# Fantom-foundation/go-txflow

Measured on AMD Instinct MI355X. Metric: verified+tallied TxVotes/sec, higher is better.
Workload: dtype u32

## Files before the change

### go-txflow_amd/csrc/fe10.h

```cpp
#pragma once
#include "fe.h"

namespace txv {

struct fe10 { uint32_t v[10]; };

#define TXV_W10(i) (((i) & 1) ? 25 : 26)
#define TXV_M10(i) (((i) & 1) ? 0x1ffffffu : 0x3ffffffu)

TXV_HD uint32_t fe10_2p(int i) { return i == 0 ? 0x7ffffdau : ((i & 1) ? 0x3fffffeu : 0x7fffffeu); }

TXV_HD fe10 fe10_zero() { fe10 r; for (int i = 0; i < 10; ++i) r.v[i] = 0; return r; }
TXV_HD fe10 fe10_one() { fe10 r = fe10_zero(); r.v[0] = 1; return r; }

TXV_HD fe10 fe10_add(const fe10& a, const fe10& b) {
  fe10 r;
#pragma unroll
  for (int i = 0; i < 10; ++i) r.v[i] = a.v[i] + b.v[i];
  return r;
}
TXV_HD fe10 fe10_sub(const fe10& a, const fe10& b) {
  fe10 r;
#pragma unroll
  for (int i = 0; i < 10; ++i) r.v[i] = (a.v[i] + fe10_2p(i)) - b.v[i];
// ... 191 lines not shown
  }
  const uint32_t t = r.v[0] + 19u * c;
  r.v[0] = t & 0x3ffffffu;
  r.v[1] += t >> 26;
  return r;
}

TXV_HD fe10 fe10_from_fe(const fe& a) {
  fe10 r;
  const uint32_t top = a.v[7] >> 31;
  int bit = 0;
#pragma unroll
  for (int i = 0; i < 10; ++i) {
    const int w = bit >> 5, s = bit & 31;
    uint32_t x = a.v[w] >> s;
    if (s + TXV_W10(i) > 32 && w < 7) x |= a.v[w + 1] << (32 - s);
    r.v[i] = x & TXV_M10(i);
    bit += TXV_W10(i);
  }
  r.v[0] += 19u * top;
  return r;
}

TXV_HD fe fe_from_fe10(const fe10& a) {
  const fe10 s = fe10_strict(a);
  fe r;
#pragma unroll
  for (int w = 0; w < 8; ++w) r.v[w] = 0;
  int bit = 0;
#pragma unroll
  for (int i = 0; i < 10; ++i) {
    const int w = bit >> 5, sh = bit & 31;
    r.v[w] |= s.v[i] << sh;
    if (sh + TXV_W10(i) > 32 && w < 7) r.v[w + 1] |= s.v[i] >> (32 - sh);
    bit += TXV_W10(i);
  }
  return r;
}

}
```

### go-txflow_amd/csrc/fe_inv_var.h

```cpp
#pragma once
#include "fe.h"

namespace txv {

struct s30 { int32_t v[9]; };

constexpr int32_t kM30 = 0x3FFFFFFF;
TXV_HD int32_t p30(int i) { return i == 0 ? 0x3FFFFFED : (i == 8 ? 0x7FFF : 0x3FFFFFFF); }
constexpr uint32_t inv30_p() {
  uint32_t p0 = 0x3FFFFFEDu, x = p0;
  for (int i = 0; i < 5; ++i) x *= 2u - p0 * x;
  return x & 0x3FFFFFFFu;
}
constexpr uint32_t kPInv30 = inv30_p();
static_assert((0x3FFFFFEDu * kPInv30 & 0x3FFFFFFFu) == 1u, "p^-1 mod 2^30");

TXV_HD uint32_t inv256_odd(uint32_t f) {
  uint32_t x = f;
  x *= 2u - f * x;
  x *= 2u - f * x;
  return x;
}

TXV_HD int32_t divsteps30_var(int32_t eta, uint32_t f, uint32_t g, int32_t t[4]) {
  uint32_t u = 1, v = 0, q = 0, r = 1;
  int i = 30;
  for (;;) {
    const int zeros = __builtin_ctz(g | (0xFFFFFFFFu << i));
    g >>= zeros; u <<= zeros; v <<= zeros; eta -= zeros; i -= zeros;
    if (i == 0) break;
    if (eta < 0) {
      uint32_t tmp;
      eta = -eta;
      tmp = f; f = g; g = 0u - tmp;
      tmp = u; u = q; q = 0u - tmp;
      tmp = v; v = r; r = 0u - tmp;
    }
    const int limit = (eta + 1) > i ? i : (eta + 1);
    const uint32_t m = (0xFFFFFFFFu >> (32 - limit)) & 255u;
    const uint32_t w = (g * inv256_odd(f)) & m;
    g -= f * w; q -= u * w; r -= v * w;
  }
// ... 100 lines not shown
```

### go-txflow_amd/csrc/ge.h

```cpp
#pragma once
#include "fe.h"
#include "fe10.h"

namespace txv {

struct ge_ext { fe X, Y, Z, T; };
struct ge_niels { fe ypx, ymx, xy2d; };

TXV_HD ge_ext ge_identity() {
  ge_ext r; r.X = fe_zero(); r.Y = fe_one(); r.Z = fe_one(); r.T = fe_zero(); return r;
}

struct ge10_ext { fe10 X, Y, Z, T; };

TXV_HD ge10_ext ge10_madd(const ge10_ext& p, const fe10& qp, const fe10& qm, const fe10& qd, bool neg) {
  const fe10 C = fe10_cneg(fe10_mul(p.T, qd), neg);
  TXV_SCHED_FENCE();
  const fe10 A = fe10_mul(fe10_sub(p.Y, p.X), qm);
  TXV_SCHED_FENCE();
  const fe10 B = fe10_mul(fe10_add(p.Y, p.X), qp);
  TXV_SCHED_FENCE();
  const fe10 E = fe10_sub(B, A), H = fe10_add(B, A);
  const fe10 G = fe10_add(p.Z, C), F = fe10_sub(p.Z, C);
  ge10_ext r;
// ... 122 lines not shown
  ge_ext r;
  r.X = fe_mul(E, F); r.Y = fe_mul(G, H); r.Z = fe_mul(F, G); r.T = fe_mul(E, H);
  return r;
}

TXV_HD ge_ext ge_dbl(const ge_ext& p) {
  fe A = fe_sq(p.X), B = fe_sq(p.Y), C = fe_dbl(fe_sq(p.Z));
  fe AB = fe_add(A, B);
  fe E = fe_sub(fe_sq(fe_add(p.X, p.Y)), AB);
  fe G = fe_sub(B, A);
  fe H = fe_neg(AB);
  fe F = fe_sub(G, C);
  ge_ext r;
  r.X = fe_mul(E, F); r.Y = fe_mul(G, H); r.Z = fe_mul(F, G); r.T = fe_mul(E, H);
  return r;
}

TXV_HD void ge_encode_zinv(uint32_t out[8], const fe& X, const fe& Y, const fe& zi) {
  fe x = fe_canon(fe_mul(X, zi));
  fe y = fe_canon(fe_mul(Y, zi));
#pragma unroll
  for (int i = 0; i < 8; ++i) out[i] = y.v[i];
  out[7] |= (x.v[0] & 1u) << 31;
}
TXV_HD void ge_encode(uint32_t out[8], const ge_ext& p) { ge_encode_zinv(out, p.X, p.Y, fe_invert(p.Z)); }

TXV_HD bool ge_decode(ge_ext& h, const uint32_t w[8]) {
  fe one = fe_one();
  h.Y = fe_from_words_255(w);
  h.Z = one;
  fe u = fe_sq(h.Y);
  fe v = fe_mul(u, fe_const_d());
  u = fe_sub(u, one);
  v = fe_add(v, one);
  fe v3 = fe_mul(fe_sq(v), v);
  fe x = fe_mul(fe_mul(fe_sq(v3), v), u);
  x = fe_pow22523(x);
  x = fe_mul(fe_mul(x, v3), u);
  fe vxx = fe_mul(fe_sq(x), v);
  bool ok = true;
  if (!fe_iszero(fe_sub(vxx, u))) {
    if (!fe_iszero(fe_add(vxx, u))) ok = false;
    x = fe_mul(x, fe_const_sqrtm1());
  }
  if (fe_parity(x) != (w[7] >> 31)) x = fe_neg(x);
  h.X = x;
// ... 15 lines not shown
```

### go-txflow_amd/csrc/kernels_verify.hip

```cpp
#include <algorithm>
#include <cstdlib>

#include "ed25519_dev.h"
#include "fe_inv_var.h"
#include "txv_device.h"

using namespace txv;

#ifndef TXV_K1A_PREFETCH
#define TXV_K1A_PREFETCH 0
#endif

#ifndef TXV_INV_VAR
#define TXV_INV_VAR 1
#endif
__device__ __forceinline__ fe verify_invert(const fe& z) {
#if TXV_INV_VAR
  return fe_invert_var(z);
#else
  return fe_invert(z);
#endif
}

template <int W>
__global__ void __launch_bounds__(64) txv_k_build_tables(const uint32_t* __restrict__ pubs_le, uint32_t n_points,
                                                          uint32_t* __restrict__ tables,
                                                          uint8_t* __restrict__ decode_ok,
                                                          uint32_t* __restrict__ addr_words,
                                                          const uint32_t* __restrict__ out_slot) {
  constexpr int chunks = (Tab<W>::kEntries - 1) / 8;
  constexpr uint64_t per_point = Tab<W>::kBuildLanes;
  const uint64_t gid = (uint64_t)blockIdx.x * 64 + threadIdx.x;
  const uint32_t pt = (uint32_t)(gid / per_point);
  const int t = (int)(gid % per_point);
  if (pt >= n_points) return;
  constexpr int last = Tab<W>::kPositions - 1;
  const bool top = Tab<W>::kLongTop && t >= last * chunks;
  const int pos = top ? last : t / chunks, c = top ? t - last * chunks : t % chunks;
  uint32_t w[8];
#pragma unroll
  for (int i = 0; i < 8; ++i) w[i] = pubs_le[pt * 8 + i];
  if (t == 0 && addr_words) {
    uint32_t h[8];
    sha256_32bytes(h, w);
#pragma unroll
// ... 59 lines not shown
                                                              uint32_t s_out[8]) {
  return vote_challenge(a, i, k_out, s_out);
}

__device__ __forceinline__ bool vote_checks(const VerifyArgs& a, uint32_t i, uint32_t s[16], uint64_t pre[8]) {
  const uint8_t fl = a.flags[i];
  const uint32_t v = a.val[i];
#pragma unroll
  for (int j = 0; j < 16; ++j) s[j] = a.sig[(size_t)j * a.n_pad + i];
  const bool bad = !(fl & TXV_FLAG_PENDING) || !(fl & TXV_FLAG_SIG64) || (fl & TXV_FLAG_BADMSG) ||
                   (s[15] & 0xE0000000u) || !a.decode_ok[v] || !sc_lt_L(s + 8);
  const uint32_t* pw = a.pubs_le + (size_t)v * 8;
#pragma unroll
  for (int j = 0; j < 4; ++j) {
    pre[j] = be64_from_le32(s[2 * j], s[2 * j + 1]);
    pre[4 + j] = be64_from_le32(pw[2 * j], pw[2 * j + 1]);
  }
  return !bad;
}

__global__ void __launch_bounds__(256, 2) txv_k_challenge2(VerifyArgs a) {
  const uint32_t half = (a.n + 1) / 2;
  const uint32_t t = blockIdx.x * 256 + threadIdx.x;
  if (t >= half) return;
  const uint32_t i0 = t, i1 = t + half;
  const bool has1 = i1 < a.n;
  uint32_t s0[16], s1[16];
  uint64_t p0[8], p1[8];
  const bool ok0 = vote_checks(a, i0, s0, p0);
  const bool ok1 = has1 && vote_checks(a, has1 ? i1 : i0, s1, p1);
  if (!ok0 && !ok1) {
    a.ok_out[i0] = 0;
    if (has1) a.ok_out[i1] = 0;
    return;
  }
  const uint32_t j1 = has1 ? i1 : i0;
  MsgView m0{a.msg + i0, a.n_pad, a.msg_words, a.msg_len[i0]};
  MsgView m1{a.msg + j1, a.n_pad, a.msg_words, a.msg_len[j1]};
  uint32_t d0[16], d1[16];
  sha512_prefixed2(d0, p0, m0, d1, p1, m1, 8);
  if (ok0) {
    const sc k = sc_reduce512(d0);
#pragma unroll
    for (int j = 0; j < 8; ++j) a.kbuf[(size_t)j * a.n_pad + i0] = k.v[j];
  }
  a.ok_out[i0] = ok0 ? 2 : 0;
  if (has1) {
    if (ok1) {
      const sc k = sc_reduce512(d1);
#pragma unroll
      for (int j = 0; j < 8; ++j) a.kbuf[(size_t)j * a.n_pad + i1] = k.v[j];
    }
    a.ok_out[i1] = ok1 ? 2 : 0;
  }
}

#ifndef TXV_K1A_WAVES
#define TXV_K1A_WAVES 4
#endif
#ifdef TXV_K1A_VGPRS
#define TXV_K1A_VGPR_ATTR __attribute__((amdgpu_num_vgpr(TXV_K1A_VGPRS)))
#else
#define TXV_K1A_VGPR_ATTR
#endif
__global__ void __launch_bounds__(256, TXV_K1A_WAVES) TXV_K1A_VGPR_ATTR txv_k_challenge(VerifyArgs a) {
  const uint32_t i = blockIdx.x * 256 + threadIdx.x;
  if (i >= a.n) return;
  if (!(a.flags[i] & TXV_FLAG_PENDING)) { a.ok_out[i] = 0; return; }
  uint32_t k[8], s[8];
  if (!vote_challenge(a, i, k, s)) { a.ok_out[i] = 0; return; }
#pragma unroll
  for (int j = 0; j < 8; ++j) a.kbuf[(size_t)j * a.n_pad + i] = k[j];
  a.ok_out[i] = 2;
}

template <int W, typename PtrB>
__device__ __forceinline__ void scalarmult_loop(const VerifyArgs& a, PtrB btab, uint32_t first, uint32_t stride) {
  for (uint32_t idx = first; idx < a.n_work; idx += stride) {
    const uint32_t i = a.order ? a.order[idx] : idx;
    if (a.ok_out[i] != 2) continue;
    const uint32_t v = a.val[i];
    uint32_t s[8], k[8];
#pragma unroll
    for (int j = 0; j < 8; ++j) { s[j] = a.sig[(size_t)(8 + j) * a.n_pad + i]; k[j] = a.kbuf[(size_t)j * a.n_pad + i]; }
    const uint32_t* ta = a.atables + (size_t)tab_slot(a, v) * Tab<W>::kWords;
    ge_ext R = double_scalarmult_w<W>(btab, ta, s, k, true);
    uint32_t enc[8];
    ge_encode_zinv(enc, R.X, R.Y, verify_invert(R.Z));
    uint32_t diff = 0;
// ... 104 lines not shown
__device__ __forceinline__ const uint4* entry_piece(const uint4* buf, int j) {
  const int e = threadIdx.x & 63;
  return buf + 64 * (e >> 3) + 8 * (e & 7) + ((j - e) & 7);
}

__device__ __forceinline__ fe10 entry_field_lds(const uint4* buf, bool neg, int role) {
  fe10 r;
  if (role == 2) {
    const uint2 d0 = reinterpret_cast<const uint2*>(entry_piece(buf, 5))[1];
    const uint4 d1 = *entry_piece(buf, 6), d2 = *entry_piece(buf, 7);
    r.v[0] = d0.x; r.v[1] = d0.y; r.v[2] = d1.x; r.v[3] = d1.y;
    r.v[4] = d1.z; r.v[5] = d1.w; r.v[6] = d2.x; r.v[7] = d2.y; r.v[8] = d2.z; r.v[9] = d2.w;
    return r;
  }
  const int j0 = (neg != (role == 1)) ? 3 : 0;
  const uint4 p0 = *entry_piece(buf, j0), p1 = *entry_piece(buf, j0 + 1);
  const uint2 p2 = *reinterpret_cast<const uint2*>(entry_piece(buf, j0 + 2));
  r.v[0] = p0.x; r.v[1] = p0.y; r.v[2] = p0.z; r.v[3] = p0.w;
  r.v[4] = p1.x; r.v[5] = p1.y; r.v[6] = p1.z; r.v[7] = p1.w; r.v[8] = p2.x; r.v[9] = p2.y;
  return r;
}

template <int WB, int WA, int PD>
__device__ __forceinline__ ge_ext double_scalarmult_pf(const uint32_t* tb, const uint32_t* ta, uint32_t va,
                                                       const uint32_t s_in[8], const uint32_t k_in[8], uint4* buf) {
  static_assert(WB >= WA, "B window must be at least the A window");
  static_assert(PD == 1 || PD == 2, "prefetch depth");
  constexpr int nB = Tab<WB>::kPositions, nA = Tab<WA>::kPositions, nT = nB + nA;
  uint32_t s[8], k[8], cs = 0, ck = 0;
#pragma unroll
  for (int i = 0; i < 8; ++i) { s[i] = s_in[i]; k[i] = k_in[i]; }
  auto issue = [&](int t) -> bool {
    const bool isB = t < 2 * nB && !(t & 1);
    const int pos = t < 2 * nB ? (t >> 1) : t - nB;
    uint4* b = buf + (PD == 2 ? (t & 1) * 512 : 0);
    if (isB) {
      const int d = next_digit<WB>(s, cs);
      entries_to_lds(tb, (uint32_t)(pos * Tab<WB>::kEntries + (d < 0 ? -d : d)), b);
      return d < 0;
    }
    const int d = table_digit<WA>(k, ck, pos);
    entries_to_lds(ta, (uint32_t)(va * (uint32_t)(Tab<WA>::kWords / kEntryWords) + pos * Tab<WA>::kEntries + (d < 0 ? -d : d)), b);
    return d > 0;
  };
  ge10_ext P;
  bool neg = issue(0), neg2 = false;
  if (PD == 2) neg2 = issue(1);
// ... 6 lines not shown
    auto next = [&]() {
      asm volatile("s_waitcnt lgkmcnt(0)" ::: "memory");
      if (PD == 2) {
        neg = neg2;
        if (t + 2 < nT) neg2 = issue(t + 2);
      } else if (t + 1 < nT) {
        neg = issue(t + 1);
      }
    };
    if (t) {
      P = ge10_madd_rd(P, [&](int role) { return entry_field_lds(bt, neg_t, role); }, neg_t, next);
    } else {
      const fe10 qp = entry_field_lds(bt, neg_t, 0), qm = entry_field_lds(bt, neg_t, 1);
      next();
      P = ge10_from_entry(qp, qm);
    }
  }
  {
    asm volatile("s_waitcnt vmcnt(0)" ::: "memory");
    const uint4* bt = buf + (PD == 2 ? ((nT - 1) & 1) * 512 : 0);
    const bool neg_t = neg;
    P = ge10_madd_rd<false>(P, [&](int role) { return entry_field_lds(bt, neg_t, role); }, neg_t, [] {});
  }
  ge_ext R;
  R.X = fe_from_fe10(P.X);
  R.Y = fe_from_fe10(P.Y);
  R.Z = fe_from_fe10(P.Z);
  R.T = fe_zero();
  return R;
}

template <int WB, int WA>
__device__ __forceinline__ ge_ext double_scalarmult_rs(const uint32_t* tb, const uint32_t* ta, uint32_t va,
                                                       const uint32_t s_in[8], const uint32_t k_in[8], uint4* buf) {
  static_assert(WB >= WA, "B window must be at least the A window");
  constexpr int nB = Tab<WB>::kPositions, nA = Tab<WA>::kPositions, nT = nB + nA;
  static_assert(nT >= 4, "schedule too short");
  uint32_t s[8], k[8], cs = 0, ck = 0;
#pragma unroll
  for (int i = 0; i < 8; ++i) { s[i] = s_in[i]; k[i] = k_in[i]; }
  auto issue = [&](int t) -> bool {
    const bool isB = t < 2 * nB && !(t & 1);
    const int pos = t < 2 * nB ? (t >> 1) : t - nB;
    uint4* b = buf + (t & 1) * 512;
    if (isB) {
      const int d = next_digit<WB>(s, cs);
      entries_to_lds(tb, (uint32_t)(pos * Tab<WB>::kEntries + (d < 0 ? -d : d)), b);
      return d < 0;
    }
    const int d = table_digit<WA>(k, ck, pos);
    entries_to_lds(ta, (uint32_t)(va * (uint32_t)(Tab<WA>::kWords / kEntryWords) + pos * Tab<WA>::kEntries + (d < 0 ? -d : d)), b);
    return d > 0;
  };
  const bool n0 = issue(0), n1a = issue(1);
  asm volatile("s_waitcnt vmcnt(8)" ::: "memory");
  fe10 qp = entry_field_lds(buf, n0, 0), qm = entry_field_lds(buf, n0, 1), qd;
// ... 27 lines not shown
      qd = entry_field_lds(bn, nq1, 2);
    }
    TXV_SCHED_FENCE();
    const fe10 E = fe10_sub(B, A), H = fe10_add(B, A);
    const fe10 G = fe10_add(P.Z, C), F = fe10_sub(P.Z, C);
    ge10_ext r;
    r.X = fe10_mul(F, E);
    TXV_SCHED_FENCE();
    if (more) {
      asm volatile("s_waitcnt lgkmcnt(0)" ::: "memory");
      ncur = nq1;
      nq1 = nq2;
      if (t + 3 < nT) nq2 = issue(t + 3);
    }
    TXV_SCHED_FENCE();
    r.Y = fe10_mul(H, G);
    TXV_SCHED_FENCE();
    r.Z = fe10_mul(F, G);
    TXV_SCHED_FENCE();
    r.T = more ? fe10_mul(H, E) : fe10_zero();
    TXV_SCHED_FENCE();
    P = r;
  }
  ge_ext R;
  R.X = fe_from_fe10(P.X);
  R.Y = fe_from_fe10(P.Y);
  R.Z = fe_from_fe10(P.Z);
  R.T = fe_zero();
  return R;
}

#ifndef TXV_K1B_REGSTAGE
#define TXV_K1B_REGSTAGE 1
#endif
template <int WB, int WA, int PD>
__device__ __forceinline__ ge_ext k1b_walk(const uint32_t* tb, const uint32_t* ta, uint32_t va, const uint32_t s[8],
                                           const uint32_t k[8], uint4* buf) {
  if constexpr (TXV_K1B_REGSTAGE && PD == 2) return double_scalarmult_rs<WB, WA>(tb, ta, va, s, k, buf);
  else return double_scalarmult_pf<WB, WA, PD>(tb, ta, va, s, k, buf);
}

#ifndef TXV_PARK_LAST
#define TXV_PARK_LAST 1
#endif
#ifndef TXV_V4_WAVES
#define TXV_V4_WAVES 2
#endif
#ifndef TXV_EXP_NO_TAIL
#define TXV_EXP_NO_TAIL 0
#endif
#ifndef TXV_EXP_NO_WALK
#define TXV_EXP_NO_WALK 0
#endif
#ifdef TXV_K1B_VGPRS
#define TXV_K1B_VGPR_ATTR __attribute__((amdgpu_num_vgpr(TXV_K1B_VGPRS)))
#else
#define TXV_K1B_VGPR_ATTR
#endif
template <int BLOCK, int WB, int WA, int V>
__global__ void __launch_bounds__(BLOCK, V == 8 ? 2 : TXV_V4_WAVES * BLOCK / 512) TXV_K1B_VGPR_ATTR txv_k_scalarmult_multi(VerifyArgs a) {
  const uint32_t n_grp = (a.n_work + 64u * V - 1u) / (64u * V) * 64u;
  const uint32_t groups = gridDim.x >= 8 ? 8u : 1u;
// ... 95 lines not shown
        inv = fe_mul(inv, Z);
      } else {
        zi = inv;
      }
      if (act >> h & 1u) {
        const uint32_t idx = (g & ~63u) * V + 64u * h + (g & 63u);
        const uint32_t i = a.order ? a.order[idx] : idx;
        uint32_t enc[8];
        ge_encode_zinv(enc, X, Y, zi);
        uint32_t diff = 0;
#pragma unroll
        for (int j = 0; j < 8; ++j) diff |= enc[j] ^ a.sig[(size_t)j * a.n_pad + i];
        a.ok_out[i] = diff == 0;
      }
    }
  }
}

#ifndef TXV_K1B_DYNAMIC
#define TXV_K1B_DYNAMIC 1
#endif
#ifndef TXV_K1B_DYN_WAVES
#define TXV_K1B_DYN_WAVES 2
#endif
template <int BLOCK, int WB, int WA, int V, int WAVES, bool FUSED>
__device__ __forceinline__ void k1b_dyn_body(const VerifyArgs& a) {
  const uint32_t lane = threadIdx.x & 63;
  const uint32_t n_chunks = (a.n_work + 63u) / 64u;
  const uint32_t xg = gridDim.x >= 8 ? 8u : 1u, myx = blockIdx.x % xg;
  const uint32_t per = (n_chunks + xg - 1u) / xg;
  const uint32_t gwave = (blockIdx.x * BLOCK + threadIdx.x) >> 6;
  uint32_t* park = a.park + (size_t)gwave * V * TXV_PARK_WORDS * 64 + lane;
  constexpr int PD = WAVES >= 3 ? 1 : 2;
  __shared__ uint4 pf[BLOCK / 64][PD * 8 * 64];
  uint4* wbuf = pf[__builtin_amdgcn_readfirstlane(threadIdx.x >> 6)];
  uint32_t src = 0;
  auto next_chunk = [&]() -> uint32_t {
    while (src < xg) {
      const uint32_t x = (myx + src) % xg;
      const uint32_t end = min(n_chunks, (x + 1u) * per);
      uint32_t c = 0;
      if (lane == 0) c = atomicAdd(a.wctr + 16u * x, 1u);
      c = x * per + __builtin_amdgcn_readfirstlane(c);
      if (c < end) return c;
      ++src;
    }
    return 0xFFFFFFFFu;
  };
  for (;;) {
    ge_ext R;
    fe P;
    uint32_t h = 0;
#pragma unroll 1
    for (; h < (uint32_t)V; ++h) {
      const uint32_t c = next_chunk();
      if (c == 0xFFFFFFFFu) break;
      const uint32_t idx = 64u * c + lane;
      const uint32_t i = idx < a.n_work ? (a.order ? a.order[idx] : idx) : 0u;
      bool on;
      uint32_t s[8], k[8];
      if constexpr (FUSED) {
        on = idx < a.n_work && (a.flags[i] & TXV_FLAG_PENDING) && vote_challenge_call(a, i, k, s);
        if (idx < a.n_work && !on) a.ok_out[i] = 0;
        if (!on) {
#pragma unroll
          for (int j = 0; j < 8; ++j) { s[j] = 0u; k[j] = 0u; }
        }
      } else {
        on = idx < a.n_work && a.ok_out[i] == 2;
#pragma unroll
        for (int j = 0; j < 8; ++j) {
          s[j] = on ? a.sig[(size_t)(8 + j) * a.n_pad + i] : 0u;
          k[j] = on ? a.kbuf[(size_t)j * a.n_pad + i] : 0u;
        }
      }
      R = k1b_walk<WB, WA, PD>(a.btable, a.atables, on ? tab_slot(a, a.val[i]) : 0u, s, k, wbuf);
      P = h ? fe_mul(P, R.Z) : R.Z;
      uint32_t* slot = park + h * TXV_PARK_WORDS * 64;
#pragma unroll
      for (int j = 0; j < 8; ++j) {
        slot[j * 64] = R.X.v[j];
        slot[(8 + j) * 64] = R.Y.v[j];
        slot[(16 + j) * 64] = P.v[j];
        slot[(24 + j) * 64] = R.Z.v[j];
      }
      slot[32 * 64] = on ? i + 1u : 0u;
    }
    if (h == 0) break;
    fe inv = verify_invert(P);
#pragma unroll 1
    for (int hh = (int)h - 1; hh >= 0; --hh) {
      const uint32_t* slot = park + hh * TXV_PARK_WORDS * 64;
      fe X, Y, Z, zi;
#pragma unroll
      for (int j = 0; j < 8; ++j) {
        X.v[j] = slot[j * 64];
        Y.v[j] = slot[(8 + j) * 64];
        Z.v[j] = slot[(24 + j) * 64];
      }
      const uint32_t i1 = slot[32 * 64];
      if (hh) {
        const uint32_t* prev = park + (hh - 1) * TXV_PARK_WORDS * 64;
        fe Pp;
#pragma unroll
        for (int j = 0; j < 8; ++j) Pp.v[j] = prev[(16 + j) * 64];
        zi = fe_mul(inv, Pp);
        inv = fe_mul(inv, Z);
      } else {
        zi = inv;
      }
      if (i1) {
        const uint32_t i = i1 - 1u;
        uint32_t enc[8];
        ge_encode_zinv(enc, X, Y, zi);
        uint32_t diff = 0;
#pragma unroll
        for (int j = 0; j < 8; ++j) diff |= enc[j] ^ a.sig[(size_t)j * a.n_pad + i];
        a.ok_out[i] = diff == 0;
      }
    }
    if (h < (uint32_t)V) break;
  }
}

template <int BLOCK, int WB, int WA, int V, int WAVES = 2>
__global__ void __launch_bounds__(BLOCK, WAVES) TXV_K1B_VGPR_ATTR txv_k_scalarmult_dyn(VerifyArgs a) {
  k1b_dyn_body<BLOCK, WB, WA, V, WAVES, false>(a);
}
#ifndef TXV_K1B_FUSED_VGPRS
#define TXV_K1B_FUSED_VGPRS 200
#endif
template <int BLOCK, int WB, int WA>
__global__ void __launch_bounds__(BLOCK, 2) __attribute__((amdgpu_num_vgpr(TXV_K1B_FUSED_VGPRS)))
txv_k_scalarmult_dyn_fused(VerifyArgs a) {
  k1b_dyn_body<BLOCK, WB, WA, 8, 2, true>(a);
}

template <int BLOCK, int WB, int WA>
__global__ void __launch_bounds__(BLOCK, 2 * BLOCK / 256) txv_k_scalarmult_points(VerifyArgs a) {
  const uint32_t n_grp = (a.n_work + 63u) & ~63u;
  const uint32_t groups = gridDim.x >= 8 ? 8u : 1u;
  const uint32_t grp = blockIdx.x % groups, blocks_in_grp = gridDim.x / groups + (grp < gridDim.x % groups);
  const uint32_t chunk = ((n_grp + groups - 1) / groups + 63u) & ~63u;
  const uint32_t lo = grp * chunk, hi = min(n_grp, lo + chunk);
// ... 420 lines not shown
  return hipSuccess;
}

template <int B, int WB, int WA>
static hipError_t launch_multi(const VerifyArgs* args, uint32_t grid, hipStream_t st) {
  if (args->lane_votes == 1) {
    if (!args->rpts) return hipErrorInvalidValue;
    if constexpr (WB >= 24) {
      static const bool split = !(getenv("TXV_K1B_SPLIT") && atoi(getenv("TXV_K1B_SPLIT")) == 0);
      if (split) {
        const uint32_t waves = (args->n_work + 15u) / 16u;
        const uint32_t blocks = std::max<uint32_t>(1, std::min<uint32_t>((waves + 3u) / 4u, std::max<uint32_t>(args->n_cus, 1u) * TXV_SPLIT_WAVES));
        hipLaunchKernelGGL((txv_k_scalarmult_split<WB, WA>), dim3(blocks), dim3(256), 0, st, *args);
        return launch_batch_encode(args, st);
      }
    }
    hipLaunchKernelGGL((txv_k_scalarmult_points<B, WB, WA>), dim3(grid), dim3(B), 0, st, *args);
    return launch_batch_encode(args, st);
  } else if (args->lane_votes == 4) {
    hipLaunchKernelGGL((txv_k_scalarmult_multi<B, WB, WA, 4>), dim3(grid), dim3(B), 0, st, *args);
  } else if (args->lane_votes == 8) {
    if constexpr (WB >= 24) {
      if (TXV_K1B_DYNAMIC && args->wctr) {
        const hipError_t e = hipMemsetAsync(args->wctr, 0, 8 * 16 * sizeof(uint32_t), st);
        if (e != hipSuccess) return e;
        if constexpr (TXV_K1B_DYN_WAVES >= 3) {
          static const int per100 = getenv("TXV_K1B_DYN_BLOCKS") ? atoi(getenv("TXV_K1B_DYN_BLOCKS")) : 100 * TXV_K1B_DYN_WAVES;
          const uint32_t want = std::max<uint32_t>(8, args->n_cus * (uint32_t)std::max(per100, 1) / 100u);
          const uint32_t grid3 = std::min<uint32_t>(want, args->park_waves / 4u);
          if (!grid3) return hipErrorInvalidValue;
          hipLaunchKernelGGL((txv_k_scalarmult_dyn<256, WB, WA, 8, TXV_K1B_DYN_WAVES>),
                             dim3(grid3), dim3(256), 0, st, *args);
        } else if (args->fused_k1a) {
          hipLaunchKernelGGL((txv_k_scalarmult_dyn_fused<B, WB, WA>), dim3(grid), dim3(B), 0, st, *args);
        } else {
          hipLaunchKernelGGL((txv_k_scalarmult_dyn<B, WB, WA, 8>), dim3(grid), dim3(B), 0, st, *args);
        }
      } else {
        hipLaunchKernelGGL((txv_k_scalarmult_multi<B, WB, WA, 8>), dim3(grid), dim3(B), 0, st, *args);
      }
    } else {
      return hipErrorInvalidValue;
    }
  } else if (args->lane_votes == 2 && WB == WA) {
    hipLaunchKernelGGL((txv_k_scalarmult_pair<B, WA>), dim3(grid), dim3(B), 0, st, *args);
  } else {
    return hipErrorInvalidValue;
  }
// ... 143 lines not shown
```

### go-txflow_amd/csrc/runtime.cpp

```cpp
#include "../../include/txvote.h"
#include "txv_device.h"
#include "txv_flow.h"
#include "amino.hpp"
#include "host_pack.hpp"
#include "sha2.h"
#include "route.h"

#include <hip/hip_runtime.h>
#include <emmintrin.h>
#include <algorithm>
#include <chrono>
#include <cstdio>
#include <cctype>
#include <cstdlib>
#include <sched.h>
#include <cstring>
#include <memory>
#include <mutex>
#include <random>
#include <system_error>
#include <thread>
#include <string>
#include <unordered_map>
#include <vector>
// ... 556 lines not shown
  a.order = by_val ? s.d_order : nullptr; a.pubs_le = pubs; a.decode_ok = dok; a.atables = tabs; a.btable = c->d_btable;
  a.ok_out = s.d_ok;
  a.tslot = tslot;
  a.park = c->d_park;
  a.park_waves = (uint32_t)(c->park_words / ((size_t)8 * TXV_PARK_WORDS * 64));
  a.n_cus = (uint32_t)c->n_cus;
  a.wctr = c->d_wctr;
  a.rpts = s.d_rpts;
  a.lane_votes = c->lane_votes;
  return a;
}

uint32_t launch_lane_votes(const txv_ctx* c, int wb, uint32_t n_work) {
  const bool wide = wb == 24 || wb == 26;
  if (c->lane_auto) return wide && n_work >= (3u << 18) ? 8u : 1u;
  if (!wide) return c->lane_votes == 8 ? 4u : c->lane_votes;
  return c->lane_votes;
}

int ensure_park(txv_ctx* c) {
  if (c->lane_votes == 1) return TXV_OK;
  const size_t words = (size_t)(c->lane_auto ? 8u : c->lane_votes) * TXV_PARK_WORDS * (size_t)c->n_cus * 2 * TXV_VERIFY_BLOCK;
  int r;
  if (!c->d_wctr && (r = dalloc(c, &c->d_wctr, 8 * 16))) return r;
  if (words <= c->park_words) return TXV_OK;
  if ((r = dalloc(c, &c->d_park, words))) return r;
  c->park_words = words;
  return TXV_OK;
}

int encode_signbytes_device(txv_ctx* c, Slot& s, const txv_votes* v, const uint8_t* d_chain, uint32_t chain_len,
                            uint64_t arena_end) {
  const uint32_t n = s.n, np = s.n_pad;
  if (arena_end + 16 > s.arena_cap) {
    int r;
    const size_t cap = std::max<size_t>((size_t)arena_end + 16, s.arena_cap * 2);
    if ((r = halloc(c, &s.h_arena, cap)) || (r = dalloc(c, &s.d_arena_th, cap))) return r;
    s.arena_cap = cap;
  }
  c->pool->parallel_for(n, [&](uint32_t lo, uint32_t hi) {
    memcpy(s.h_fh + lo, v->height + lo, (size_t)(hi - lo) * 8);
    memcpy(s.h_fs + lo, v->ts_sec + lo, (size_t)(hi - lo) * 8);
    memcpy(s.h_fn + lo, v->ts_nanos + lo, (size_t)(hi - lo) * 4);
    memcpy(s.h_fo + lo, v->txhash_off + lo, (size_t)(hi - lo) * 4);
    memcpy(s.h_fl + lo, v->txhash_len + lo, (size_t)(hi - lo) * 4);
  }, 16384);
  if (arena_end) memcpy(s.h_arena, v->txhash, (size_t)arena_end);
// ... 291 lines not shown
  hipStream_t ps = c->key_stream;
  HIP_TRY(c, hipStreamWaitEvent(ps, s.ev[3], 0));
  if (s.launched) HIP_TRY(c, hipStreamWaitEvent(ps, s.ev[4], 0));
  if (s.fill_mask || s.fill_key) {
    if ((r = slot_fills(c, s, ps))) return r;
    HIP_TRY(c, hipEventRecord(s.ev[3], ps));
  }
  HIP_TRY(c, hipStreamWaitEvent(c->stream, s.ev[3], 0));
  static const bool prep_after = getenv("TXV_PREP_AFTER_K1B") && atoi(getenv("TXV_PREP_AFTER_K1B")) == 1;
  if (prep_after && c->vend_n >= 2) HIP_TRY(c, hipStreamWaitEvent(ps, c->vend_ev[(c->vend_n - 2) % 4], 0));
  HIP_TRY(c, hipEventRecord(s.ev[0], ps));
  SignBytesArgs sa{};
  sa.n = s.n; sa.n_pad = s.n_pad; sa.msg_words = s.msg_words; sa.chain_len = fb.chain_len;
  sa.height = s.d_fh; sa.ts_sec = s.d_fs; sa.ts_nanos = s.d_fn; sa.txhash_off = s.d_fo; sa.txhash_len = s.d_fl;
  sa.txhash = s.d_arena_th; sa.chain = c->d_chain; sa.msg_len = nullptr; sa.nil = s.has_nil ? s.d_nil : nullptr;
  sa.msg = s.d_msg;
  VerifyArgs va = verify_args(c, s, c->d_pubs, c->d_decode_ok, c->d_atables, c->tab_w, c->d_vslot);
  va.order = nullptr;
  va.n_work = s.n;
  va.lane_votes = launch_lane_votes(c, c->b_w, va.n_work);
  if (!txv_verify_windows_supported(c->b_w, c->tab_w)) { c->err = "verify windows"; return TXV_EDEVICE; }
  static const bool fuse = getenv("TXV_K1B_FUSED") && atoi(getenv("TXV_K1B_FUSED")) == 1;
  va.fused_k1a = fuse && txv_k1b_fusable(c->b_w, &va) ? 1u : 0u;
  HIP_TRY(c, txv_flow_prep(&fs, &fb, ps));
  HIP_TRY(c, txv_launch_signbytes(&sa, ps));
  if (TXV_K1A_ON_KEY_STREAM && !va.fused_k1a) {
    HIP_TRY(c, hipEventRecord(s.ev[8], ps));
    HIP_TRY(c, txv_launch_challenge(&va, ps));
  }
  HIP_TRY(c, hipEventRecord(s.ev[1], ps));
  HIP_TRY(c, hipStreamWaitEvent(c->vstream, s.ev[1], 0));
  HIP_TRY(c, hipEventRecord(s.ev[7], c->vstream));
  static const bool after_tally = getenv("TXV_K1B_AFTER_TALLY") && atoi(getenv("TXV_K1B_AFTER_TALLY")) == 1;
  if (!TXV_K1A_ON_KEY_STREAM || va.fused_k1a) {
    if (!va.fused_k1a) HIP_TRY(c, txv_launch_challenge(&va, c->vstream));
    if (after_tally && c->tally_ev_set) HIP_TRY(c, hipStreamWaitEvent(c->vstream, c->tally_ev, 0));
    HIP_TRY(c, hipEventRecord(s.ev[8], c->vstream));
  }
  HIP_TRY(c, txv_launch_scalarmult(c->b_w, c->tab_w, &va, verify_grid(c, s.n), c->vstream));
  HIP_TRY(c, hipEventRecord(s.ev[2], c->vstream));
  if (prep_after) {
    hipEvent_t& ve = c->vend_ev[c->vend_n % 4];
    if (!ve) HIP_TRY(c, hipEventCreateWithFlags(&ve, hipEventDisableTiming));
    HIP_TRY(c, hipEventRecord(ve, c->vstream));
    ++c->vend_n;
  }
// ... 3328 lines not shown
```

### go-txflow_amd/csrc/txv_device.h

```cpp
#pragma once
#include <stdint.h>
#include <hip/hip_runtime.h>

#ifndef TXV_VERIFY_BLOCK
#define TXV_VERIFY_BLOCK 512
#endif

#define TXV_FLAG_PENDING 0x01u
#define TXV_FLAG_SIG64   0x02u
#define TXV_FLAG_BADMSG  0x04u

struct VerifyArgs {
  uint32_t n, n_pad, msg_words, n_work;
  uint32_t* kbuf;
  const uint32_t* sig;
  const uint64_t* msg;
  const uint32_t* msg_len;
  const uint32_t* val;
  const uint8_t* flags;
  const uint32_t* order;
  const uint32_t* pubs_le;
  const uint8_t* decode_ok;
  const uint32_t* atables;
  const uint32_t* btable;
  uint8_t* ok_out;
  uint32_t* park;
  uint32_t lane_votes;
  uint32_t* rpts;
  uint32_t* wctr;
  uint32_t park_waves;
  uint32_t n_cus;
  uint32_t fused_k1a;
  const uint32_t* tslot;
};

#define TXV_PARK_WORDS 33
#define TXV_MAX_LANE_VOTES 4
#define TXV_RPTS_WORDS 32

struct SignBytesArgs {
  uint32_t n, n_pad, msg_words, chain_len;
  const int64_t* height;
  const int64_t* ts_sec;
  const int32_t* ts_nanos;
  const uint32_t* txhash_off;
  const uint32_t* txhash_len;
  const uint8_t* txhash;
  const uint8_t* chain;
  const uint32_t* msg_len;
  const uint8_t* nil;
  uint64_t* msg;
};

struct SignArgs {
  uint32_t n, n_pad, msg_words, pad0;
  const uint64_t* msg;
  const uint32_t* msg_len;
  const uint32_t* val;
  const uint32_t* prefix;
// ... 58 lines not shown
```

Baseline: 785.8 million.

## Keep batched-inversion park state in radix-2^25.5 limbs and fold wctr zeroing into k1a

The dynamic k1b verify path now parks X, Y, the running product and Z in 10-limb fe10 form instead of converting to 8-word packed form after each scalar walk. The Montgomery batch-inversion walk-back and the point encoding are done with paired fe10 multiplies, and a lighter canonicalisation replaces the full conversion before encoding. This removes per-vote fe conversions and lets two multiplies issue together, at the cost of a larger park buffer (41 words instead of 33) and more memory traffic per slot. It also zeroes the work counter inside the challenge kernel instead of issuing a separate hipMemsetAsync, shortens the Newton seed in inv256_odd, and adds an optional block-wide inversion path that is off by default.

```diff
diff --git a/go-txflow_amd/csrc/fe10.h b/go-txflow_amd/csrc/fe10.h
--- a/go-txflow_amd/csrc/fe10.h
+++ b/go-txflow_amd/csrc/fe10.h
@@ -237,8 +237,22 @@
   return r;
 }
 
-TXV_HD fe fe_from_fe10(const fe10& a) {
-  const fe10 s = fe10_strict(a);
+TXV_HD fe10 fe10_canon(const fe10& a) {
+  uint32_t q = (a.v[0] + 19u) >> 26;
+#pragma unroll
+  for (int i = 1; i < 10; ++i) q = (a.v[i] + q) >> TXV_W10(i);
+  fe10 r;
+  uint32_t c = 19u * q;
+#pragma unroll
+  for (int i = 0; i < 10; ++i) {
+    const uint32_t t = a.v[i] + c;
+    c = t >> TXV_W10(i);
+    r.v[i] = t & TXV_M10(i);
+  }
+  return r;
+}
+
+TXV_HD fe fe_pack_fe10(const fe10& s) {
   fe r;
 #pragma unroll
   for (int w = 0; w < 8; ++w) r.v[w] = 0;
@@ -253,4 +267,6 @@
   return r;
 }
 
-}
+TXV_HD fe fe_from_fe10(const fe10& a) { return fe_pack_fe10(fe10_strict(a)); }
+
+}
diff --git a/go-txflow_amd/csrc/fe_inv_var.h b/go-txflow_amd/csrc/fe_inv_var.h
--- a/go-txflow_amd/csrc/fe_inv_var.h
+++ b/go-txflow_amd/csrc/fe_inv_var.h
@@ -16,8 +16,7 @@
 static_assert((0x3FFFFFEDu * kPInv30 & 0x3FFFFFFFu) == 1u, "p^-1 mod 2^30");
 
 TXV_HD uint32_t inv256_odd(uint32_t f) {
-  uint32_t x = f;
-  x *= 2u - f * x;
+  uint32_t x = (f + (f << 1)) ^ 2u;
   x *= 2u - f * x;
   return x;
 }
diff --git a/go-txflow_amd/csrc/ge.h b/go-txflow_amd/csrc/ge.h
--- a/go-txflow_amd/csrc/ge.h
+++ b/go-txflow_amd/csrc/ge.h
@@ -168,6 +168,20 @@
 #pragma unroll
   for (int i = 0; i < 8; ++i) out[i] = y.v[i];
   out[7] |= (x.v[0] & 1u) << 31;
+}
+TXV_HD void ge10_encode_zinv(uint32_t out[8], const fe10& X, const fe10& Y, const fe10& zi) {
+  fe10 x, y;
+  fe10_mul2(X, zi, Y, zi, x, y);
+  const fe yw = fe_pack_fe10(fe10_canon(y));
+#pragma unroll
+  for (int i = 0; i < 8; ++i) out[i] = yw.v[i];
+  out[7] |= (fe10_canon(x).v[0] & 1u) << 31;
+}
+TXV_HD fe10 fe10_walk_back(fe10& inv, const fe10& Pprev, const fe10& Z) {
+  fe10 zi, up;
+  fe10_mul2(inv, Pprev, inv, Z, zi, up);
+  inv = up;
+  return zi;
 }
 TXV_HD void ge_encode(uint32_t out[8], const ge_ext& p) { ge_encode_zinv(out, p.X, p.Y, fe_invert(p.Z)); }
 
diff --git a/go-txflow_amd/csrc/k1b_tail.h b/go-txflow_amd/csrc/k1b_tail.h
--- /dev/null
+++ b/go-txflow_amd/csrc/k1b_tail.h
@@ -0,0 +1,56 @@
+#pragma once
+#include "fe10.h"
+
+namespace txv {
+
+constexpr uint32_t kXchgP = 0, kXchgInv = 10, kXchgQ = 20, kXchgWords = 30;
+
+TXV_HD fe10 xchg_load(const uint32_t* area, uint32_t field, uint32_t lane) {
+  fe10 r;
+#pragma unroll
+  for (int j = 0; j < 10; ++j) r.v[j] = area[(field + j) * 64 + lane];
+  return r;
+}
+TXV_HD void xchg_store(uint32_t* area, uint32_t field, uint32_t lane, const fe10& x) {
+#pragma unroll
+  for (int j = 0; j < 10; ++j) area[(field + j) * 64 + lane] = x.v[j];
+}
+
+template <int NW, typename Invert>
+TXV_HD void k1b_block_invert(uint32_t* base, uint32_t stride, uint32_t lane, uint32_t took, Invert invert) {
+  fe10 Q;
+  bool first = true;
+#if defined(__HIP_DEVICE_COMPILE__)
+#pragma unroll 1
+#endif
+  for (int w = 0; w < NW; ++w) {
+    if (!(took >> w & 1u)) continue;
+    uint32_t* area = base + (size_t)w * stride;
+    const fe10 Pw = xchg_load(area, kXchgP, lane);
+    Q = first ? Pw : fe10_mul(Q, Pw);
+    first = false;
+    xchg_store(area, kXchgQ, lane, Q);
+  }
+  fe10 inv = invert(Q);
+#if defined(__HIP_DEVICE_COMPILE__)
+#pragma unroll 1
+#endif
+  for (int w = NW - 1; w >= 0; --w) {
+    if (!(took >> w & 1u)) continue;
+    uint32_t* area = base + (size_t)w * stride;
+    const uint32_t below = took & ((1u << w) - 1u);
+    if (below) {
+      const int pw = 31 - __builtin_clz(below);
+      const fe10 Qp = xchg_load(base + (size_t)pw * stride, kXchgQ, lane);
+      const fe10 Pw = xchg_load(area, kXchgP, lane);
+      fe10 iw, up;
+      fe10_mul2(inv, Qp, inv, Pw, iw, up);
+      xchg_store(area, kXchgInv, lane, iw);
+      inv = up;
+    } else {
+      xchg_store(area, kXchgInv, lane, inv);
+    }
+  }
+}
+
+}
diff --git a/go-txflow_amd/csrc/kernels_verify.hip b/go-txflow_amd/csrc/kernels_verify.hip
--- a/go-txflow_amd/csrc/kernels_verify.hip
+++ b/go-txflow_amd/csrc/kernels_verify.hip
@@ -3,6 +3,7 @@
 
 #include "ed25519_dev.h"
 #include "fe_inv_var.h"
+#include "k1b_tail.h"
 #include "txv_device.h"
 
 using namespace txv;
@@ -21,6 +22,8 @@
   return fe_invert(z);
 #endif
 }
+
+__device__ __forceinline__ fe10 verify_invert10(const fe10& z) { return fe10_from_fe(verify_invert(fe_from_fe10(z))); }
 
 template <int W>
 __global__ void __launch_bounds__(64) txv_k_build_tables(const uint32_t* __restrict__ pubs_le, uint32_t n_points,
@@ -126,6 +129,7 @@
 __global__ void __launch_bounds__(256, 2) txv_k_challenge2(VerifyArgs a) {
   const uint32_t half = (a.n + 1) / 2;
   const uint32_t t = blockIdx.x * 256 + threadIdx.x;
+  if (a.k1a_zeroes_wctr && t < 8u) a.wctr[16u * t] = 0u;
   if (t >= half) return;
   const uint32_t i0 = t, i1 = t + half;
   const bool has1 = i1 < a.n;
@@ -169,6 +173,7 @@
 #endif
 __global__ void __launch_bounds__(256, TXV_K1A_WAVES) TXV_K1A_VGPR_ATTR txv_k_challenge(VerifyArgs a) {
   const uint32_t i = blockIdx.x * 256 + threadIdx.x;
+  if (a.k1a_zeroes_wctr && i < 8u) a.wctr[16u * i] = 0u;
   if (i >= a.n) return;
   if (!(a.flags[i] & TXV_FLAG_PENDING)) { a.ok_out[i] = 0; return; }
   uint32_t k[8], s[8];
@@ -319,7 +324,7 @@
 }
 
 template <int WB, int WA, int PD>
-__device__ __forceinline__ ge_ext double_scalarmult_pf(const uint32_t* tb, const uint32_t* ta, uint32_t va,
+__device__ __forceinline__ ge10_ext double_scalarmult_pf10(const uint32_t* tb, const uint32_t* ta, uint32_t va,
                                                        const uint32_t s_in[8], const uint32_t k_in[8], uint4* buf) {
   static_assert(WB >= WA, "B window must be at least the A window");
   static_assert(PD == 1 || PD == 2, "prefetch depth");
@@ -372,6 +377,9 @@
     const bool neg_t = neg;
     P = ge10_madd_rd<false>(P, [&](int role) { return entry_field_lds(bt, neg_t, role); }, neg_t, [] {});
   }
+  return P;
+}
+__device__ __forceinline__ ge_ext ge_from_walk10(const ge10_ext& P) {
   ge_ext R;
   R.X = fe_from_fe10(P.X);
   R.Y = fe_from_fe10(P.Y);
@@ -379,9 +387,14 @@
   R.T = fe_zero();
   return R;
 }
+template <int WB, int WA, int PD>
+__device__ __forceinline__ ge_ext double_scalarmult_pf(const uint32_t* tb, const uint32_t* ta, uint32_t va,
+                                                       const uint32_t s_in[8], const uint32_t k_in[8], uint4* buf) {
+  return ge_from_walk10(double_scalarmult_pf10<WB, WA, PD>(tb, ta, va, s_in, k_in, buf));
+}
 
 template <int WB, int WA>
-__device__ __forceinline__ ge_ext double_scalarmult_rs(const uint32_t* tb, const uint32_t* ta, uint32_t va,
+__device__ __forceinline__ ge10_ext double_scalarmult_rs10(const uint32_t* tb, const uint32_t* ta, uint32_t va,
                                                        const uint32_t s_in[8], const uint32_t k_in[8], uint4* buf) {
   static_assert(WB >= WA, "B window must be at least the A window");
   constexpr int nB = Tab<WB>::kPositions, nA = Tab<WA>::kPositions, nT = nB + nA;
@@ -455,22 +468,22 @@
     TXV_SCHED_FENCE();
     P = r;
   }
-  ge_ext R;
-  R.X = fe_from_fe10(P.X);
-  R.Y = fe_from_fe10(P.Y);
-  R.Z = fe_from_fe10(P.Z);
-  R.T = fe_zero();
-  return R;
+  return P;
 }
 
 #ifndef TXV_K1B_REGSTAGE
 #define TXV_K1B_REGSTAGE 1
 #endif
+template <int WB, int WA, int PD>
+__device__ __forceinline__ ge10_ext k1b_walk10(const uint32_t* tb, const uint32_t* ta, uint32_t va, const uint32_t s[8],
+                                               const uint32_t k[8], uint4* buf) {
+  if constexpr (TXV_K1B_REGSTAGE && PD == 2) return double_scalarmult_rs10<WB, WA>(tb, ta, va, s, k, buf);
+  else return double_scalarmult_pf10<WB, WA, PD>(tb, ta, va, s, k, buf);
+}
 template <int WB, int WA, int PD>
 __device__ __forceinline__ ge_ext k1b_walk(const uint32_t* tb, const uint32_t* ta, uint32_t va, const uint32_t s[8],
                                            const uint32_t k[8], uint4* buf) {
-  if constexpr (TXV_K1B_REGSTAGE && PD == 2) return double_scalarmult_rs<WB, WA>(tb, ta, va, s, k, buf);
-  else return double_scalarmult_pf<WB, WA, PD>(tb, ta, va, s, k, buf);
+  return ge_from_walk10(k1b_walk10<WB, WA, PD>(tb, ta, va, s, k, buf));
 }
 
 #ifndef TXV_PARK_LAST
@@ -612,6 +625,9 @@
 #endif
 #ifndef TXV_K1B_DYN_WAVES
 #define TXV_K1B_DYN_WAVES 2
+#endif
+#ifndef TXV_K1B_BLOCK_INV
+#define TXV_K1B_BLOCK_INV 0
 #endif
 template <int BLOCK, int WB, int WA, int V, int WAVES, bool FUSED>
 __device__ __forceinline__ void k1b_dyn_body(const VerifyArgs& a) {
@@ -638,8 +654,6 @@
     return 0xFFFFFFFFu;
   };
   for (;;) {
-    ge_ext R;
-    fe P;
     uint32_t h = 0;
 #pragma unroll 1
     for (; h < (uint32_t)V; ++h) {
@@ -664,52 +678,88 @@
           k[j] = on ? a.kbuf[(size_t)j * a.n_pad + i] : 0u;
         }
       }
-      R = k1b_walk<WB, WA, PD>(a.btable, a.atables, on ? tab_slot(a, a.val[i]) : 0u, s, k, wbuf);
-      P = h ? fe_mul(P, R.Z) : R.Z;
+      const ge10_ext R = k1b_walk10<WB, WA, PD>(a.btable, a.atables, on ? tab_slot(a, a.val[i]) : 0u, s, k, wbuf);
       uint32_t* slot = park + h * TXV_PARK_WORDS * 64;
-#pragma unroll
-      for (int j = 0; j < 8; ++j) {
+      fe10 P = R.Z;
+      if (h) {
+        fe10 Pp;
+#pragma unroll
+        for (int j = 0; j < 10; ++j) Pp.v[j] = (slot - TXV_PARK_WORDS * 64)[(20 + j) * 64];
+        P = fe10_mul(Pp, R.Z);
+      }
+#pragma unroll
+      for (int j = 0; j < 10; ++j) {
         slot[j * 64] = R.X.v[j];
-        slot[(8 + j) * 64] = R.Y.v[j];
-        slot[(16 + j) * 64] = P.v[j];
-        slot[(24 + j) * 64] = R.Z.v[j];
-      }
-      slot[32 * 64] = on ? i + 1u : 0u;
-    }
+        slot[(10 + j) * 64] = R.Y.v[j];
+        slot[(20 + j) * 64] = P.v[j];
+        slot[(30 + j) * 64] = R.Z.v[j];
+      }
+      slot[40 * 64] = on ? i + 1u : 0u;
+    }
+    fe10 P, inv;
+    if (h) {
+#pragma unroll
+      for (int j = 0; j < 10; ++j) P.v[j] = park[((h - 1) * TXV_PARK_WORDS + 20 + j) * 64];
+    }
+#if TXV_K1B_BLOCK_INV
+    constexpr int NW = BLOCK / 64;
+    constexpr uint32_t stride = PD * 8 * 64 * 4;
+    static_assert(kXchgWords * 64 + 1 <= stride, "exchange area fits a wave's gather buffer");
+    uint32_t* xbase = reinterpret_cast<uint32_t*>(&pf[0][0]);
+    const uint32_t wave = __builtin_amdgcn_readfirstlane(threadIdx.x >> 6);
+    uint32_t* xmine = xbase + wave * stride;
+    if (h) xchg_store(xmine, kXchgP, lane, P);
+    if (lane == 0) xmine[kXchgWords * 64] = h;
+    __syncthreads();
+    uint32_t took = 0, full = 0;
+#pragma unroll 1
+    for (int w = 0; w < NW; ++w) {
+      const uint32_t hw = __builtin_amdgcn_readfirstlane(xbase[w * stride + kXchgWords * 64]);
+      took |= (hw ? 1u : 0u) << w;
+      full |= hw == (uint32_t)V;
+    }
+    if (!took) break;
+    if (wave == 0) k1b_block_invert<NW>(xbase, stride, lane, took, [](const fe10& z) { return verify_invert10(z); });
+    __syncthreads();
+    if (h) inv = xchg_load(xmine, kXchgInv, lane);
+#else
     if (h == 0) break;
-    fe inv = verify_invert(P);
+    inv = verify_invert10(P);
+#endif
 #pragma unroll 1
     for (int hh = (int)h - 1; hh >= 0; --hh) {
       const uint32_t* slot = park + hh * TXV_PARK_WORDS * 64;
-      fe X, Y, Z, zi;
-#pragma unroll
-      for (int j = 0; j < 8; ++j) {
+      fe10 X, Y, zi;
+#pragma unroll
+      for (int j = 0; j < 10; ++j) {
         X.v[j] = slot[j * 64];
-        Y.v[j] = slot[(8 + j) * 64];
-        Z.v[j] = slot[(24 + j) * 64];
-      }
-      const uint32_t i1 = slot[32 * 64];
+        Y.v[j] = slot[(10 + j) * 64];
+      }
+      const uint32_t i1 = slot[40 * 64];
       if (hh) {
         const uint32_t* prev = park + (hh - 1) * TXV_PARK_WORDS * 64;
-        fe Pp;
-#pragma unroll
-        for (int j = 0; j < 8; ++j) Pp.v[j] = prev[(16 + j) * 64];
-        zi = fe_mul(inv, Pp);
-        inv = fe_mul(inv, Z);
+        fe10 Pp, Z;
+#pragma unroll
+        for (int j = 0; j < 10; ++j) { Pp.v[j] = prev[(20 + j) * 64]; Z.v[j] = slot[(30 + j) * 64]; }
+        zi = fe10_walk_back(inv, Pp, Z);
       } else {
         zi = inv;
       }
       if (i1) {
         const uint32_t i = i1 - 1u;
         uint32_t enc[8];
-        ge_encode_zinv(enc, X, Y, zi);
+        ge10_encode_zinv(enc, X, Y, zi);
         uint32_t diff = 0;
 #pragma unroll
         for (int j = 0; j < 8; ++j) diff |= enc[j] ^ a.sig[(size_t)j * a.n_pad + i];
         a.ok_out[i] = diff == 0;
       }
     }
+#if TXV_K1B_BLOCK_INV
+    if (!full) break;
+#else
     if (h < (uint32_t)V) break;
+#endif
   }
 }
 
@@ -1176,8 +1226,10 @@
   } else if (args->lane_votes == 8) {
     if constexpr (WB >= 24) {
       if (TXV_K1B_DYNAMIC && args->wctr) {
-        const hipError_t e = hipMemsetAsync(args->wctr, 0, 8 * 16 * sizeof(uint32_t), st);
-        if (e != hipSuccess) return e;
+        if (!args->k1a_zeroes_wctr) {
+          const hipError_t e = hipMemsetAsync(args->wctr, 0, 8 * 16 * sizeof(uint32_t), st);
+          if (e != hipSuccess) return e;
+        }
         if constexpr (TXV_K1B_DYN_WAVES >= 3) {
           static const int per100 = getenv("TXV_K1B_DYN_BLOCKS") ? atoi(getenv("TXV_K1B_DYN_BLOCKS")) : 100 * TXV_K1B_DYN_WAVES;
           const uint32_t want = std::max<uint32_t>(8, args->n_cus * (uint32_t)std::max(per100, 1) / 100u);
diff --git a/go-txflow_amd/csrc/runtime.cpp b/go-txflow_amd/csrc/runtime.cpp
--- a/go-txflow_amd/csrc/runtime.cpp
+++ b/go-txflow_amd/csrc/runtime.cpp
@@ -602,7 +602,10 @@
   if (c->lane_votes == 1) return TXV_OK;
   const size_t words = (size_t)(c->lane_auto ? 8u : c->lane_votes) * TXV_PARK_WORDS * (size_t)c->n_cus * 2 * TXV_VERIFY_BLOCK;
   int r;
-  if (!c->d_wctr && (r = dalloc(c, &c->d_wctr, 8 * 16))) return r;
+  if (!c->d_wctr) {
+    if ((r = dalloc(c, &c->d_wctr, 8 * 16))) return r;
+    HIP_TRY(c, hipMemset(c->d_wctr, 0, 8 * 16 * sizeof(uint32_t)));
+  }
   if (words <= c->park_words) return TXV_OK;
   if ((r = dalloc(c, &c->d_park, words))) return r;
   c->park_words = words;
@@ -940,6 +943,7 @@
   if (!txv_verify_windows_supported(c->b_w, c->tab_w)) { c->err = "verify windows"; return TXV_EDEVICE; }
   static const bool fuse = getenv("TXV_K1B_FUSED") && atoi(getenv("TXV_K1B_FUSED")) == 1;
   va.fused_k1a = fuse && txv_k1b_fusable(c->b_w, &va) ? 1u : 0u;
+  va.k1a_zeroes_wctr = !TXV_K1A_ON_KEY_STREAM && !va.fused_k1a && va.wctr ? 1u : 0u;
   HIP_TRY(c, txv_flow_prep(&fs, &fb, ps));
   HIP_TRY(c, txv_launch_signbytes(&sa, ps));
   if (TXV_K1A_ON_KEY_STREAM && !va.fused_k1a) {
diff --git a/go-txflow_amd/csrc/txv_device.h b/go-txflow_amd/csrc/txv_device.h
--- a/go-txflow_amd/csrc/txv_device.h
+++ b/go-txflow_amd/csrc/txv_device.h
@@ -31,10 +31,11 @@
   uint32_t park_waves;
   uint32_t n_cus;
   uint32_t fused_k1a;
+  uint32_t k1a_zeroes_wctr;
   const uint32_t* tslot;
 };
 
-#define TXV_PARK_WORDS 33
+#define TXV_PARK_WORDS 41
 #define TXV_MAX_LANE_VOTES 4
 #define TXV_RPTS_WORDS 32
 
```

After: 783.7 million. About the same (-0.3%).
